# houzhijian/CONE

Measured on AMD Instinct MI355X. Metric: windows/sec + queries/sec, Ego4D-NLQ win_len=90 d=256 top-k=20, higher is better.
Workload: dtype f32

## Files before the change

cone_amd/csrc/ffn.hip:

```cpp
#include <mutex>

#include "tail_f32_common.h"

namespace cone {

constexpr int FFN_STAGE = 2 * 16 * 256;
constexpr int FFN_NST = 4;

template <bool PROJ, bool QKV, int NW, bool PRE = false>
__global__ __launch_bounds__(64 * NW, NW / 4) void ffn_fused_kernel(FfnArgs p) {
    static_assert(!PRE || (PROJ && !QKV), "the pre-norm form is the layer tail");
    constexpr int FFN_ROWS = 16 * NW, FFN_NPIECE = 32 / NW, NT = 64 * NW, HW = NW / 2;
    extern __shared__ __attribute__((aligned(16))) float smem[];
    float* b1s = smem + FFN_NST * FFN_STAGE;
    TF_LAUNCH_ROWS(M, p, 0)
    const int n_tiles = (M + FFN_ROWS - 1) / FFN_ROWS;
    if (n_tiles == 0) return;
    const int G_ = (int)gridDim.x;
    const int full_items = ((n_tiles - 1) / G_) * G_;
    const int rem_rows = M - full_items * FFN_ROWS;
    const int rem_half = (rem_rows + 63) >> 6;
    const bool half_mode = NW == 8 && rem_half <= G_ && 2 * ((rem_rows + FFN_ROWS - 1) / FFN_ROWS) <= G_;
    const int n_items = full_items + (half_mode ? rem_half : (rem_rows + FFN_ROWS - 1) / FFN_ROWS);
    if ((int)blockIdx.x >= n_items) return;
    const int tid = threadIdx.x, lane = tid & 63;
    const int wave = __builtin_amdgcn_readfirstlane(tid >> 6);
    auto wave_row0 = [&](int it) -> int {
        if (it < full_items || !half_mode) return it * FFN_ROWS + wave * 16;
        return wave < 4 ? full_items * FFN_ROWS + (it - full_items) * 64 + wave * 16 : M;
    };
    const int li = lane & 15, lg = lane >> 4;
    const int ff = p.ff, nc = ff >> 4;
    constexpr int NP = PROJ ? 8 : 0;
    const int NQ = QKV ? p.n_qkv >> 5 : 0;
    const int G = NP + nc + NQ;

    float* prm = b1s + ff;
    for (int i = tid; i < (ff >> 2); i += NT)
        reinterpret_cast<f32x4*>(b1s)[i] = reinterpret_cast<const f32x4*>(p.b1)[i];
    if (tid < 64) {
        reinterpret_cast<f32x4*>(prm)[tid] = reinterpret_cast<const f32x4*>(p.b2)[tid];
        reinterpret_cast<f32x4*>(prm + 256)[tid] = reinterpret_cast<const f32x4*>(p.ln_g)[tid];
        reinterpret_cast<f32x4*>(prm + 512)[tid] = reinterpret_cast<const f32x4*>(p.ln_b)[tid];
        if (PROJ) {
            reinterpret_cast<f32x4*>(prm + 768)[tid] = reinterpret_cast<const f32x4*>(p.bo)[tid];
            reinterpret_cast<f32x4*>(prm + 1024)[tid] = reinterpret_cast<const f32x4*>(p.pg)[tid];
            reinterpret_cast<f32x4*>(prm + 1280)[tid] = reinterpret_cast<const f32x4*>(p.pb)[tid];
        }
    }
    float* qbs = prm + 1536;
    if (QKV)
        for (int i = tid; i < (p.n_qkv >> 2); i += NT)
            reinterpret_cast<f32x4*>(qbs)[i] = reinterpret_cast<const f32x4*>(p.qb)[i];

    const int drow = lane >> 2;
    const int dch = (lane & 3) ^ tf_swz16(drow);
    const bool w2side = wave >= HW;
    const float* fbase = w2side ? p.W2 : p.W1;
    const int foff = w2side ? (16 * FFN_NPIECE * (wave - HW) + drow) * ff + 4 * dch
                            : drow * 256 + 16 * FFN_NPIECE * wave + 4 * dch;
    const int fpiece = w2side ? 16 * ff : 16;
    const int fchunk = w2side ? 16 : 16 * 256;
    const int poff = PROJ ? (16 * (wave / HW) + drow) * 256 + 16 * FFN_NPIECE * (wave % HW) + 4 * dch : 0;
    int sb = 0;
    auto stream_piece = [&](int g, int i) {
        float* dstp = smem + ((sb + g) % FFN_NST) * FFN_STAGE + (wave * FFN_NPIECE + i) * 256;
        const int gg = g < G ? g : g - G;
        const bool qk = QKV && gg >= NP + nc;
        const bool pj = (PROJ && gg < NP) || qk;
        const char* ub = reinterpret_cast<const char*>(
            qk ? p.Wq + ((size_t)(gg - NP - nc) * (32 * 256) + 16 * i)
               : (pj ? p.Wo + ((size_t)gg * (32 * 256) + 16 * i) : fbase + ((size_t)(gg - NP) * fchunk + (size_t)i * fpiece)));
        const unsigned vo = (unsigned)((pj ? poff : foff) * 4);
        asm volatile("" : "+s"(ub));
        TF_GLDS16(ub + vo, dstp);
    };

    const int rd = li * 16 + ((lg ^ tf_swz16(li)) << 2);
#define FFN_RD(stg, off) (*reinterpret_cast<const f32x4*>((stg) + (off) + rd))
#define FFN_STAGE_OF(g) (smem + ((sb + (g)) % FFN_NST) * FFN_STAGE)
#define FFN_SB() __builtin_amdgcn_sched_barrier(0)
#define FFN_STREAM(g, u) { if (FFN_NPIECE == 8) stream_piece(g, u); else if ((u) & 1) stream_piece(g, (u) >> 1); }
#define FFN_END_CHUNK()                                                           \
    {                                                                             \
        FFN_SB();                                                                 \
        asm volatile("s_waitcnt vmcnt(%0)" ::"n"(FFN_NPIECE) : "memory");         \
        __builtin_amdgcn_s_barrier();                                             \
        FFN_SB();                                                                 \
    }
#define FFN_MFMA(acc, a, b) { acc = __builtin_amdgcn_mfma_f32_16x16x4f32(a, b, acc, 0, 0, 0); FFN_SB(); }
#define FFN_MM_A(acc, w0, w1, B, q)                                                   \
    {                                                                                 \
        _Pragma("unroll") for (int r = 0; r < 4; ++r) FFN_MFMA(acc[r], w0[r], B[q][r])         \
        _Pragma("unroll") for (int r = 0; r < 4; ++r) FFN_MFMA(acc[r], w1[r], B[(q) + 1][r])   \
    }
#define FFN_MM_Y(w0, w1, hh, t)                                                       \
    {                                                                                 \
        _Pragma("unroll") for (int r = 0; r < 4; ++r) {                               \
            FFN_MFMA(y[t], w0[r], hh[r])                                              \
            FFN_MFMA(y[(t) + 1], w1[r], hh[r])                                        \
        }                                                                             \
    }
#define FFN_MM_AY(acc, w0, w1, B, q, v0, v1, hh, t)                                   \
    {                                                                                 \
        _Pragma("unroll") for (int r = 0; r < 4; ++r) {                               \
            FFN_MFMA(acc[r], w0[r], B[q][r])                                          \
            FFN_MFMA(y[(t) + (r & 1)], ((r & 1) ? v1 : v0)[r >> 1], hh[r >> 1])       \
        }                                                                             \
        _Pragma("unroll") for (int r = 0; r < 4; ++r) {                               \
            FFN_MFMA(acc[r], w1[r], B[(q) + 1][r])                                    \
            FFN_MFMA(y[(t) + (r & 1)], ((r & 1) ? v1 : v0)[2 + (r >> 1)], hh[2 + (r >> 1)]) \
        }                                                                             \
    }

#define FFN_CHUNK32(gi, B)                                                                                                 \
    const float* st = FFN_STAGE_OF(gi);                                                                                    \
    f32x4 ha[2], hb[2];                                                                                                    \
    ha[0] = f32x4{0.f, 0.f, 0.f, 0.f}; hb[0] = ha[0];                                                                      \
    ha[1] = ha[0]; hb[1] = ha[0];                                                                                          \
    wa = FFN_RD(st, 0); wb = FFN_RD(st, 256); va = FFN_RD(st, 4096); vb = FFN_RD(st, 4096 + 256);                          \
    _Pragma("unroll") for (int u = 0; u < 8; ++u) {                                                                        \
        FFN_SB();                                                                                                          \
        asm volatile("" : "+v"(wa), "+v"(wb), "+v"(va), "+v"(vb));                                                         \
        FFN_SB();                                                                                                          \
        if (u < 7) {                                                                                                       \
            na = FFN_RD(st, (2 * u + 2) * 256); nb = FFN_RD(st, (2 * u + 3) * 256);                                        \
            nva = FFN_RD(st, 4096 + (2 * u + 2) * 256); nvb = FFN_RD(st, 4096 + (2 * u + 3) * 256);                        \
        }                                                                                                                  \
        FFN_SB();                                                                                                          \
        _Pragma("unroll") for (int r = 0; r < 4; ++r) {                                                                    \
            FFN_MFMA(ha[r & 1], wa[r], B[2 * u][r])                                                                        \
            FFN_MFMA(hb[r & 1], va[r], B[2 * u][r])                                                                        \
        }                                                                                                                  \
        _Pragma("unroll") for (int r = 0; r < 4; ++r) {                                                                    \
            FFN_MFMA(ha[r & 1], wb[r], B[2 * u + 1][r])                                                                    \
            FFN_MFMA(hb[r & 1], vb[r], B[2 * u + 1][r])                                                                    \
        }                                                                                                                  \
        FFN_STREAM((gi) + 2, u)                                     \
        if (u < 7) { wa = na; wb = nb; va = nva; vb = nvb; }                                                               \
    }

#pragma unroll
    for (int i = 0; i < FFN_NPIECE; ++i) stream_piece(0, i);
#pragma unroll
    for (int i = 0; i < FFN_NPIECE; ++i) stream_piece(1 < G ? 1 : 0, i);

    f32x4 wa, wb, na, nb;
    f32x4 va, vb, nva, nvb;

    f32x4 xr[16];
    f32x4 ar[PROJ ? 16 : 1];
    auto load_tile = [&](int tile) {
        const int row = wave_row0(tile) + li;
        const size_t ld_row = TF_LD_ROW(row, M);
        if (PROJ) {
            const float* ap = p.A + ld_row * p.lda + 4 * lg;
#pragma unroll
            for (int q = 0; q < 16; ++q) ar[q] = *reinterpret_cast<const f32x4*>(ap + 16 * q);
        } else {
            const float* xp = p.X + ld_row * p.ldx + 4 * lg;
#pragma unroll
            for (int q = 0; q < 16; ++q) xr[q] = *reinterpret_cast<const f32x4*>(xp + 16 * q);
        }
    };
    auto load_res = [&](int tile) {
        const int row = wave_row0(tile) + li;
        const size_t ld_row = TF_LD_ROW(row, M);
        TF_RES_ROW(rp, p, ld_row, 4 * lg)
#pragma unroll
        for (int q = 0; q < 16; ++q) xr[q] = *reinterpret_cast<const f32x4*>(rp + 16 * q);
    };
    load_tile(blockIdx.x);
    bool first = true;
    for (int tile = blockIdx.x; tile < n_items; tile += gridDim.x) {
    const int my_row0 = wave_row0(tile);
    const int my_row = my_row0 + li;
    const bool act = my_row0 < M;
    if (first) {
        asm volatile("s_waitcnt vmcnt(%0)" ::"n"(FFN_NPIECE) : "memory");
        __syncthreads();
        first = false;
    }
    if (!act) {
        for (int g = 0; g < G; ++g) {
#pragma unroll
            for (int i = 0; i < FFN_NPIECE; ++i) stream_piece(g + 2, i);
            FFN_END_CHUNK()
        }
        break;
    }

    f32x4 y[16];
    if (PROJ) {
        load_res(tile);
#pragma unroll
        for (int g = 0; g < NP; ++g) {
            FFN_CHUNK32(g, ar)
            xr[2 * g] += ha[0] + ha[1];
            xr[2 * g + 1] += hb[0] + hb[1];
            FFN_END_CHUNK()
        }
        FFN_SB();
#pragma unroll
        for (int t = 0; t < 16; ++t) xr[t] += *reinterpret_cast<const f32x4*>(prm + 768 + 16 * t + 4 * lg);
        if (PRE) {
#pragma unroll
            for (int t = 0; t < 16; ++t) y[t] = xr[t] + *reinterpret_cast<const f32x4*>(prm + 16 * t + 4 * lg);
        }
        float rstd;
        tf_layernorm_regs(xr, rstd);
        TF_LN_APPLY(xr, rstd, prm + 1024, prm + 1280)
        FFN_SB();
    }

    if (!PRE) {
#pragma unroll
        for (int t = 0; t < 16; ++t) y[t] = f32x4{0.f, 0.f, 0.f, 0.f};
    }
    f32x4 h, hp[4];
    {
        const float* st = FFN_STAGE_OF(NP);
#pragma unroll
        for (int r = 0; r < 4; ++r) hp[r] = f32x4{0.f, 0.f, 0.f, 0.f};
        wa = FFN_RD(st, 0); wb = FFN_RD(st, 256);
#pragma unroll
        for (int u = 0; u < 8; ++u) {
            FFN_SB();
            asm volatile("" : "+v"(wa), "+v"(wb));
            FFN_SB();
            if (u < 7) { na = FFN_RD(st, (2 * u + 2) * 256); nb = FFN_RD(st, (2 * u + 3) * 256); }
            else { va = FFN_RD(st, 4096); vb = FFN_RD(st, 4096 + 256); }
            FFN_SB();
            FFN_MM_A(hp, wa, wb, xr, 2 * u)
            FFN_STREAM(NP + 2, u)
            if (u < 7) { wa = na; wb = nb; }
        }
        FFN_SB();
        h = (hp[0] + hp[1]) + (hp[2] + hp[3]) + *reinterpret_cast<const f32x4*>(b1s + 4 * lg);
#pragma unroll
        for (int r = 0; r < 4; ++r) h[r] = fmaxf(h[r], 0.f);
        FFN_END_CHUNK()
    }
    for (int i = 1; i < nc; ++i) {
        const float* s1 = FFN_STAGE_OF(NP + i);
        const float* s2 = FFN_STAGE_OF(NP + i - 1);
#pragma unroll
        for (int r = 0; r < 4; ++r) hp[r] = f32x4{0.f, 0.f, 0.f, 0.f};
        wa = FFN_RD(s1, 0); wb = FFN_RD(s1, 256);
#pragma unroll
        for (int u = 0; u < 8; ++u) {
            FFN_SB();
            if (u == 0) {
                asm volatile("" : "+v"(va), "+v"(vb));
                FFN_SB();
                nva = FFN_RD(s2, 4096 + 2 * 256); nvb = FFN_RD(s2, 4096 + 3 * 256);
                FFN_SB();
                FFN_MM_Y(va, vb, h, 0)
                FFN_SB();
                asm volatile("" : "+v"(wa), "+v"(wb));
                FFN_SB();
                na = FFN_RD(s1, 2 * 256); nb = FFN_RD(s1, 3 * 256);
                FFN_SB();
                FFN_MM_A(hp, wa, wb, xr, 0)
            } else {
                asm volatile("" : "+v"(wa), "+v"(wb), "+v"(va), "+v"(vb));
                FFN_SB();
                if (u < 7) {
                    na = FFN_RD(s1, (2 * u + 2) * 256); nb = FFN_RD(s1, (2 * u + 3) * 256);
                    nva = FFN_RD(s2, 4096 + (2 * u + 2) * 256); nvb = FFN_RD(s2, 4096 + (2 * u + 3) * 256);
                } else {
                    nva = FFN_RD(s1, 4096); nvb = FFN_RD(s1, 4096 + 256);
                }
                FFN_SB();
                FFN_MM_AY(hp, wa, wb, xr, 2 * u, va, vb, h, 2 * u)
            }
            FFN_STREAM(NP + i + 2, u)
            if (u < 7) { wa = na; wb = nb; }
            va = nva; vb = nvb;
        }
        FFN_SB();
        h = (hp[0] + hp[1]) + (hp[2] + hp[3]) + *reinterpret_cast<const f32x4*>(b1s + 16 * i + 4 * lg);
#pragma unroll
        for (int r = 0; r < 4; ++r) h[r] = fmaxf(h[r], 0.f);
        FFN_END_CHUNK()
    }
    {
        const float* st = FFN_STAGE_OF(NP + nc - 1);
#pragma unroll
        for (int u = 0; u < 8; ++u) {
            FFN_SB();
            asm volatile("" : "+v"(va), "+v"(vb));
            FFN_SB();
            if (u < 7) { nva = FFN_RD(st, 4096 + (2 * u + 2) * 256); nvb = FFN_RD(st, 4096 + (2 * u + 3) * 256); }
            FFN_SB();
            FFN_MM_Y(va, vb, h, 2 * u)
            if (u < 7) { va = nva; vb = nvb; }
        }
    }
    FFN_SB();
    if (!PRE) {
#pragma unroll
        for (int t = 0; t < 16; ++t) y[t] = y[t] + *reinterpret_cast<const f32x4*>(prm + 16 * t + 4 * lg) + xr[t];
    }
    FFN_SB();
    load_tile(tile + (int)gridDim.x < n_items ? tile + (int)gridDim.x : tile);
    FFN_SB();
    if (PRE && my_row < M) {
        float* op = p.OUT + (size_t)my_row * p.ldo + 4 * lg;
#pragma unroll
        for (int t = 0; t < 16; ++t) *reinterpret_cast<f32x4*>(op + 16 * t) = y[t];
    }
    float rstd;
    if (!PRE || p.OUT2) tf_layernorm_regs(y, rstd);
    if (PRE) {
        if (p.OUT2 && my_row < M) {
            float* op = p.OUT2 + (size_t)my_row * p.ldo2 + 4 * lg;
            TF_LN_STORE(op, y, rstd, prm + 256, prm + 512, true, false)
        }
    } else if (my_row < M) {
        float* op = p.OUT + (size_t)my_row * p.ldo + 4 * lg;
        TF_LN_STORE(op, y, rstd, prm + 256, prm + 512, true, QKV)
    } else if (QKV) {
#pragma unroll
        for (int t = 0; t < 16; ++t) y[t] = f32x4{0.f, 0.f, 0.f, 0.f};
    }
    if (QKV) {
        float* qrow = p.QKV + (size_t)my_row * p.ldq + 4 * lg;
        for (int g = 0; g < NQ; ++g) {
            FFN_CHUNK32(NP + nc + g, y)
            FFN_SB();
            if (my_row < M) {
                *reinterpret_cast<f32x4*>(qrow + 32 * g) = (ha[0] + ha[1]) + *reinterpret_cast<const f32x4*>(qbs + 32 * g + 4 * lg);
                *reinterpret_cast<f32x4*>(qrow + 32 * g + 16) = (hb[0] + hb[1]) + *reinterpret_cast<const f32x4*>(qbs + 32 * g + 16 + 4 * lg);
            }
            FFN_END_CHUNK()
        }
    }
    sb = (sb + G) % FFN_NST;
    }
    asm volatile("s_waitcnt vmcnt(0)" ::: "memory");
}

#undef FFN_CHUNK32
#undef FFN_MM_A
#undef FFN_MM_Y
#undef FFN_MM_AY
#undef FFN_MFMA
#undef FFN_END_CHUNK
#undef FFN_SB
#undef FFN_STREAM
#undef FFN_STAGE_OF
#undef FFN_RD

bool ffn_fused_supported(int ff) { return ff >= 32 && ff % 16 == 0 && ff <= 4096; }

bool ffn_fused_qkv_fits(int ff, int n_qkv) {
    return ffn_fused_supported(ff) && n_qkv >= 32 && n_qkv % 32 == 0 &&
           (size_t)(FFN_NST * FFN_STAGE + ff + 6 * 256 + n_qkv) * sizeof(float) <= 160 * 1024;
}

static int ffn_cu_count(int* n_cu) {
    static DeviceOnce once;
    CONE_CHECK_HIP(device_once(once, [] { return hipSuccess; }, n_cu));
    return 0;
}

template <bool PROJ, bool QKV, int NW, bool PRE = false>
static int launch_ffn_nw(const TailF32Args& a, int n_cu, hipStream_t s) {
    const size_t lds = (size_t)(FFN_NST * FFN_STAGE + a.ff + 6 * 256 + (QKV ? a.n_qkv : 0)) * sizeof(float);
    CONE_REQUIRE(lds <= 160 * 1024, "fused layer tail: %zu bytes of LDS (ff %d, q|k|v %d) exceed 160 KiB", lds, a.ff, a.n_qkv);
    static DeviceOnce once;
    int dev_cu = 0;
    CONE_CHECK_HIP(device_once(once, [] {
        return hipFuncSetAttribute((const void*)ffn_fused_kernel<PROJ, QKV, NW, PRE>, hipFuncAttributeMaxDynamicSharedMemorySize,
                                   160 * 1024);
    }, &dev_cu));
    if (!n_cu) n_cu = dev_cu;
    const int tiles = (a.M + 16 * NW - 1) / (16 * NW);
    const int grid = tiles < n_cu ? tiles : n_cu;
    ProfScope ps(NW == 8 ? (PROJ ? PK_FFN_PROJ : PK_FFN_FUSED) : (PROJ ? PK_FFN_PROJ_NW4 : PK_FFN_FUSED_NW4), a.M,
                 a.ff + (QKV ? a.n_qkv / 2 : 0), 256, a.M_dev, s);
    FfnArgs k;
    static_cast<TailF32Args&>(k) = a;
    hipLaunchKernelGGL((ffn_fused_kernel<PROJ, QKV, NW, PRE>), dim3((unsigned)grid), dim3(64 * NW), lds, s, k);
    CONE_LAUNCH_CHECK();
    return 0;
}

static int launch_ffn_rows(const TailF32Args& a, bool proj, bool pre, int nw, int n_cu, hipStream_t s) {
    if (pre) return launch_ffn_nw<true, false, 8, true>(a, n_cu, s);
    if (a.Wq) return launch_ffn_nw<true, true, 8>(a, n_cu, s);
    if (nw == 4) return proj ? launch_ffn_nw<true, false, 4>(a, n_cu, s) : launch_ffn_nw<false, false, 4>(a, n_cu, s);
    return proj ? launch_ffn_nw<true, false, 8>(a, n_cu, s) : launch_ffn_nw<false, false, 8>(a, n_cu, s);
}

#ifndef CONE_FFN_SPLIT_GROUPS
#define CONE_FFN_SPLIT_GROUPS 512
#endif
static int ffn_full_round_rows(int M, int n_cu, int ff) {
    const int tiles = (M + 127) / 128;
    if (tiles <= n_cu || !ffn_wide_supported(ff)) return M;
    const int64_t full = (int64_t)(tiles / n_cu) * n_cu * 128;
    const int64_t rem = M - full;
    return rem > 0 && (rem + 15) / 16 <= CONE_FFN_SPLIT_GROUPS ? (int)full : M;
}

static int launch_ffn_ladder(TailF32Args a, bool proj, int n_cu, int wide_groups, hipStream_t s) {
    const int M = a.M;
    const bool ride = a.Wq != nullptr;
    if (!ride && (M + 15) / 16 <= wide_groups && ffn_wide_supported(a.ff)) return launch_tail_f32_wide(a, proj, false, s);
    if (!n_cu)
        if (int rc = ffn_cu_count(&n_cu)) return rc;
    const int m1 = ride ? M : ffn_full_round_rows(M, n_cu, a.ff);
    a.M = m1;
    if (int rc = launch_ffn_rows(a, proj, false, !ride && 2 * ((m1 + 127) / 128) <= n_cu ? 4 : 8, n_cu, s)) return rc;
    if (m1 == M) return 0;
    a.M = M - m1; a.m_off = m1; a.OUT += (size_t)m1 * a.ldo;
    if (!proj) a.X += (size_t)m1 * a.ldx;
    else {
        a.A += (size_t)m1 * a.lda;
        if (a.r_idx) a.r_idx += m1; else a.R += (size_t)m1 * a.ldr;
    }
    return launch_tail_f32_wide(a, proj, false, s);
}

int launch_ffn_fused(const float* X, int ldx, const float* W1, const float* b1, const float* W2, const float* b2,
                     const float* ln_g, const float* ln_b, float* OUT, int ldo, int M, const int* M_dev, int ff,
                     hipStream_t s) {
    CONE_REQUIRE(ffn_fused_supported(ff), "fused FFN: dim_feedforward=%d unsupported", ff);
    CONE_REQUIRE(X && W1 && b1 && W2 && b2 && ln_g && ln_b && OUT, "fused FFN: null argument");
    CONE_REQUIRE(ldx % 4 == 0 && ldo % 4 == 0, "fused FFN: row strides must be multiples of 4");
    if (M <= 0) return 0;
    TailF32Args a{};
    a.X = X; a.ldx = ldx; a.W1 = W1; a.b1 = b1; a.W2 = W2; a.b2 = b2; a.ln_g = ln_g; a.ln_b = ln_b;
    a.OUT = OUT; a.ldo = ldo; a.M = M; a.M_dev = M_dev; a.ff = ff;
    return launch_ffn_ladder(a, false, 0, FFN_WIDE_GROUPS, s);
}

int launch_proj_ffn_fused(const TailArgs& t, hipStream_t s) {
    if (int rc = tail_f32_check(t, TF_FORM_ROWS, "fused layer tail")) return rc;
    if (t.M <= 0) return 0;
    return launch_ffn_ladder(tail_f32_args(t), true, 0, FFN_WIDE_GROUPS, s);
}

int launch_proj_ffn_prenorm(const TailArgs& t, hipStream_t s) {
    if (int rc = tail_f32_check(t, TF_FORM_ROWS, "pre-norm layer tail")) return rc;
    if (t.M <= 0) return 0;
    return launch_ffn_rows(tail_f32_args(t), true, true, 8, 0, s);
}

int launch_tail_f32_form(const TailArgs& t, int form, int n_cu, hipStream_t s) {
    if (form == CONE_TAIL_FORM_SPREAD) return launch_proj_ffn_spread(t, s);
    CONE_REQUIRE(form >= CONE_TAIL_FORM_ROWS128 && form <= CONE_TAIL_FORM_LADDER, "tail form hook: unknown form %d", form);
    CONE_REQUIRE(!t.pre || (form != CONE_TAIL_FORM_ROWS64 && form != CONE_TAIL_FORM_LADDER), "tail form hook: no such pre-norm form");
    CONE_REQUIRE(form != CONE_TAIL_FORM_LADDER || n_cu > 0, "tail form hook: the ladder needs a CU count");
    if (int rc = tail_f32_check(t, form == CONE_TAIL_FORM_WIDE ? TF_FORM_WIDE : TF_FORM_ROWS, "tail form hook")) return rc;
    if (t.M <= 0) return 0;
    const TailF32Args a = tail_f32_args(t);
    if (form == CONE_TAIL_FORM_WIDE) return launch_tail_f32_wide(a, true, t.pre, s);
    if (form == CONE_TAIL_FORM_LADDER) return launch_ffn_ladder(a, true, n_cu, 0, s);
    return launch_ffn_rows(a, true, t.pre, form == CONE_TAIL_FORM_ROWS64 ? 4 : 8, 0, s);
}
}
```

cone_amd/csrc/tail_f32_common.h:

```cpp
#pragma once

#include "common.h"

namespace cone {

#define TF_GLDS16(src, dst) \
    __builtin_amdgcn_global_load_lds((const __attribute__((address_space(1))) void*)(src), \
                                     (__attribute__((address_space(3))) void*)(dst), 16, 0, 0)

__device__ __forceinline__ int tf_swz16(int row) { return (0x1230 >> (((row >> 2) & 3) * 4)) & 3; }

__device__ __forceinline__ void tf_layernorm_regs(f32x4 (&v)[16], float& rstd) {
    float s1 = 0.f;
#pragma unroll
    for (int t = 0; t < 16; ++t) s1 += (v[t][0] + v[t][1]) + (v[t][2] + v[t][3]);
    s1 += __shfl_xor(s1, 16, 64);
    s1 += __shfl_xor(s1, 32, 64);
    const float mean = s1 * (1.0f / 256.0f);
    float s2 = 0.f;
#pragma unroll
    for (int t = 0; t < 16; ++t) {
#pragma unroll
        for (int r = 0; r < 4; ++r) { v[t][r] -= mean; s2 = fmaf(v[t][r], v[t][r], s2); }
    }
    s2 += __shfl_xor(s2, 16, 64);
    s2 += __shfl_xor(s2, 32, 64);
    rstd = 1.0f / sqrtf(s2 * (1.0f / 256.0f) + 1e-5f);
}
#define TF_LN_TILE(o, v, rstd, gp, bp, t)                                                       \
    {                                                                                           \
        const f32x4 g_ = *reinterpret_cast<const f32x4*>((gp) + 16 * (t) + 4 * lg);             \
        const f32x4 b_ = *reinterpret_cast<const f32x4*>((bp) + 16 * (t) + 4 * lg);             \
        _Pragma("unroll") for (int r = 0; r < 4; ++r) o[r] = v[t][r] * rstd * g_[r] + b_[r];    \
    }
#define TF_LN_APPLY(v, rstd, gp, bp) \
    _Pragma("unroll") for (int t = 0; t < 16; ++t) TF_LN_TILE(v[t], v, rstd, gp, bp, t)
#define TF_LN_STORE(op, v, rstd, gp, bp, WHEN, KEEP)             \
    _Pragma("unroll") for (int t = 0; t < 16; ++t) {             \
        if (WHEN) {                                              \
            f32x4 o_;                                            \
            TF_LN_TILE(o_, v, rstd, gp, bp, t)                   \
            *reinterpret_cast<f32x4*>((op) + 16 * t) = o_;       \
            if (KEEP) v[t] = o_;                                 \
        }                                                        \
    }

#define TF_LAUNCH_ROWS(M, p, m_off) \
    int M = (p).M;                  \
    if ((p).M_dev) { const int md_ = *(p).M_dev - (m_off); M = md_ < M ? md_ : M; }
#define TF_LD_ROW(row, M) ((size_t)((row) < (M) ? (row) : (M) - 1))
#define TF_RES_ROW(rp, p, ld_row, off)                                                                               \
    const float* rp = (p).R + (ld_row) * (p).ldr + (off);                                                            \
    if ((p).r_idx) {                                                                                                 \
        const int ix_ = (p).r_idx[ld_row];                                                                           \
        rp = (ix_ >= 0 ? (p).R + (size_t)ix_ * (p).ldr : (p).R2 + (size_t)(~ix_) * (p).ldr) + (off);                 \
    }

struct TailF32Args {
    const float* X; int ldx;
    const float* W1; const float* b1;
    const float* W2; const float* b2;
    const float* ln_g; const float* ln_b;
    float* OUT; int ldo;
    int M; const int* M_dev;
    int ff;
    const float* A; int lda; const float* R; int ldr;
    const float* Wo; const float* bo; const float* pg; const float* pb;
    const int* r_idx; const float* R2;
    const float* Wq; const float* qb; float* QKV; int ldq; int n_qkv;
    float* OUT2; int ldo2;
    int m_off;
};
struct FfnArgs : TailF32Args {};
struct FfnWideArgs : TailF32Args {};

enum { TF_FORM_ROWS = 0, TF_FORM_WIDE = 1, TF_FORM_SPREAD = 2 };

bool ffn_fused_supported(int ff);
bool ffn_wide_supported(int ff);
bool ffn_spread_supported(int M, int ff);

static inline bool tail_f32_rides(const TailArgs& t) { return !t.pre && t.next && t.next->Wq; }

static inline TailF32Args tail_f32_args(const TailArgs& t) {
    const TailWeights& w = *t.w;
    TailF32Args a{};
    a.A = t.A; a.lda = t.lda; a.Wo = w.Wo; a.bo = w.bo; a.R = t.R; a.ldr = t.ldr; a.pg = w.in_g; a.pb = w.in_b;
    a.r_idx = t.r_idx; a.R2 = t.R2;
    a.W1 = w.W1; a.b1 = w.b1; a.W2 = w.W2; a.b2 = w.b2;
    a.ln_g = t.pre && !w.out_g ? w.in_g : w.out_g; a.ln_b = t.pre && !w.out_b ? w.in_b : w.out_b;
    a.OUT = t.OUT; a.ldo = t.ldo; a.M = t.M; a.M_dev = t.M_dev; a.ff = t.ff; a.m_off = t.m_off;
    if (t.pre) { a.OUT2 = t.OUT2; a.ldo2 = t.ldo2; }
    if (tail_f32_rides(t)) { a.Wq = t.next->Wq; a.qb = t.next->qb; a.QKV = t.QKV; a.ldq = t.ldq; a.n_qkv = t.n_qkv; }
    return a;
}

static inline int tail_f32_check(const TailArgs& t, int form, const char* what) {
    const TailWeights& w = *t.w;
    CONE_REQUIRE(form != TF_FORM_SPREAD || (ffn_spread_supported(t.M, t.ff) && t.scratch), "%s: unsupported size M=%d ff=%d", what,
                 t.M, t.ff);
    CONE_REQUIRE(!t.r_idx || t.R2, "%s: a gathered residual needs both source matrices", what);
    CONE_REQUIRE(form == TF_FORM_SPREAD || (form == TF_FORM_WIDE ? ffn_wide_supported(t.ff) : ffn_fused_supported(t.ff)),
                 "%s: dim_feedforward=%d unsupported", what, t.ff);
    CONE_REQUIRE(t.A && w.Wo && w.bo && t.R && w.in_g && w.in_b && w.W1 && w.b1 && w.W2 && w.b2 && t.OUT &&
                     (t.pre ? !t.OUT2 || (w.out_g && w.out_b) : w.out_g && w.out_b), "%s: null argument", what);
    CONE_REQUIRE(t.lda % 4 == 0 && t.ldr % 4 == 0 && t.ldo % 4 == 0 && (!t.pre || !t.OUT2 || t.ldo2 % 4 == 0),
                 "%s: row strides must be multiples of 4", what);
    CONE_REQUIRE(form != TF_FORM_ROWS || !tail_f32_rides(t) ||
                     (t.next->qb && t.QKV && t.n_qkv >= 32 && t.n_qkv % 32 == 0 && t.ldq % 4 == 0), "%s: bad q|k|v arguments", what);
    return 0;
}

int launch_tail_f32_wide(const TailF32Args& a, bool proj, bool pre, hipStream_t s);
int launch_tail_f32_spread(const TailF32Args& a, bool pre, float* scratch, hipStream_t s);

}
```

Measured before the change: 375,000.

## Prefetch activation and residual rows with counted vmcnt waits in fused FFN

Row loads for the attention output, residual and input now go through inline global_load asm, and the kernel waits on them with explicit vmcnt counts that leave younger stores and weight streams in flight. The residual gather index is fetched together with the attention rows, and the next tile's attention load is issued earlier for the non-QKV projection path. The intent is to overlap these row loads with the MFMA chunks instead of stalling on full waits. The q|k|v ride path drops to a single accumulator pair. Compile-time ablation macros that disable output stores are added but default off. The hand-counted vmcnt values are fragile: a miscount could read data before it lands.

```diff
diff --git a/cone_amd/csrc/ffn.hip b/cone_amd/csrc/ffn.hip
--- a/cone_amd/csrc/ffn.hip
+++ b/cone_amd/csrc/ffn.hip
@@ -3,6 +3,20 @@
 #include "tail_f32_common.h"
 
 namespace cone {
+
+#ifndef CONE_FFN_ABL_NO_OUT_STORES
+#define CONE_FFN_ABL_NO_OUT_STORES 0
+#endif
+#ifndef CONE_FFN_ABL_NO_RIDE_STORES
+#define CONE_FFN_ABL_NO_RIDE_STORES 0
+#endif
+#ifndef CONE_FFN_STRICT_WAIT
+#define CONE_FFN_STRICT_WAIT 0
+#endif
+constexpr bool FFN_ABL_NO_OUT_STORES = CONE_FFN_ABL_NO_OUT_STORES, FFN_ABL_NO_RIDE_STORES = CONE_FFN_ABL_NO_RIDE_STORES,
+               FFN_STRICT_WAIT = CONE_FFN_STRICT_WAIT;
+#define FFN_OUT_ST(p) (!FFN_ABL_NO_OUT_STORES || (p).ldo < 0)
+#define FFN_RIDE_ST(p) (!FFN_ABL_NO_RIDE_STORES || (p).ldq < 0)
 
 constexpr int FFN_STAGE = 2 * 16 * 256;
 constexpr int FFN_NST = 4;
@@ -81,12 +95,13 @@
 #define FFN_STAGE_OF(g) (smem + ((sb + (g)) % FFN_NST) * FFN_STAGE)
 #define FFN_SB() __builtin_amdgcn_sched_barrier(0)
 #define FFN_STREAM(g, u) { if (FFN_NPIECE == 8) stream_piece(g, u); else if ((u) & 1) stream_piece(g, (u) >> 1); }
-#define FFN_END_CHUNK()                                                           \
-    {                                                                             \
-        FFN_SB();                                                                 \
-        asm volatile("s_waitcnt vmcnt(%0)" ::"n"(FFN_NPIECE) : "memory");         \
-        __builtin_amdgcn_s_barrier();                                             \
-        FFN_SB();                                                                 \
+#define FFN_END_CHUNK(younger)                                                              \
+    {                                                                                       \
+        static_assert(FFN_NPIECE + (younger) <= 63, "vmcnt is a 6-bit field");              \
+        FFN_SB();                                                                           \
+        asm volatile("s_waitcnt vmcnt(%0)" ::"n"(FFN_NPIECE + (younger)) : "memory");       \
+        __builtin_amdgcn_s_barrier();                                                       \
+        FFN_SB();                                                                           \
     }
 #define FFN_MFMA(acc, a, b) { acc = __builtin_amdgcn_mfma_f32_16x16x4f32(a, b, acc, 0, 0, 0); FFN_SB(); }
 #define FFN_MM_A(acc, w0, w1, B, q)                                                   \
@@ -113,11 +128,10 @@
         }                                                                             \
     }
 
-#define FFN_CHUNK32(gi, B)                                                                                                 \
+#define FFN_CHUNK32(gi, B, NCH)                                                                                            \
     const float* st = FFN_STAGE_OF(gi);                                                                                    \
-    f32x4 ha[2], hb[2];                                                                                                    \
-    ha[0] = f32x4{0.f, 0.f, 0.f, 0.f}; hb[0] = ha[0];                                                                      \
-    ha[1] = ha[0]; hb[1] = ha[0];                                                                                          \
+    f32x4 ha[NCH], hb[NCH];                                                                                                \
+    _Pragma("unroll") for (int c_ = 0; c_ < (NCH); ++c_) { ha[c_] = f32x4{0.f, 0.f, 0.f, 0.f}; hb[c_] = ha[c_]; }          \
     wa = FFN_RD(st, 0); wb = FFN_RD(st, 256); va = FFN_RD(st, 4096); vb = FFN_RD(st, 4096 + 256);                          \
     _Pragma("unroll") for (int u = 0; u < 8; ++u) {                                                                        \
         FFN_SB();                                                                                                          \
@@ -129,12 +143,12 @@
         }                                                                                                                  \
         FFN_SB();                                                                                                          \
         _Pragma("unroll") for (int r = 0; r < 4; ++r) {                                                                    \
-            FFN_MFMA(ha[r & 1], wa[r], B[2 * u][r])                                                                        \
-            FFN_MFMA(hb[r & 1], va[r], B[2 * u][r])                                                                        \
+            FFN_MFMA(ha[r & ((NCH) - 1)], wa[r], B[2 * u][r])                                                              \
+            FFN_MFMA(hb[r & ((NCH) - 1)], va[r], B[2 * u][r])                                                              \
         }                                                                                                                  \
         _Pragma("unroll") for (int r = 0; r < 4; ++r) {                                                                    \
-            FFN_MFMA(ha[r & 1], wb[r], B[2 * u + 1][r])                                                                    \
-            FFN_MFMA(hb[r & 1], vb[r], B[2 * u + 1][r])                                                                    \
+            FFN_MFMA(ha[r & ((NCH) - 1)], wb[r], B[2 * u + 1][r])                                                          \
+            FFN_MFMA(hb[r & ((NCH) - 1)], vb[r], B[2 * u + 1][r])                                                          \
         }                                                                                                                  \
         FFN_STREAM((gi) + 2, u)                                     \
         if (u < 7) { wa = na; wb = nb; va = nva; vb = nvb; }                                                               \
@@ -148,36 +162,55 @@
     f32x4 wa, wb, na, nb;
     f32x4 va, vb, nva, nvb;
 
+    constexpr int ROWS = 16, OUT_ST = FFN_ABL_NO_OUT_STORES ? 0 : 16, RIDE_ST = FFN_ABL_NO_RIDE_STORES ? 0 : 2;
+    constexpr int AR_WAIT = FFN_STRICT_WAIT ? 0 : OUT_ST + (QKV ? FFN_NPIECE + RIDE_ST : 0);
+    constexpr int XR_WAIT = FFN_STRICT_WAIT ? 0 : PROJ ? FFN_NPIECE : OUT_ST;
+    constexpr int END0_YOUNGER = FFN_STRICT_WAIT || PROJ ? 0 : OUT_ST;
+    constexpr int RIDE_YOUNGER = FFN_STRICT_WAIT ? 0 : 2 * RIDE_ST, RIDE0_YOUNGER = FFN_STRICT_WAIT ? 0 : ROWS + OUT_ST + RIDE_ST;
     f32x4 xr[16];
     f32x4 ar[PROJ ? 16 : 1];
-    auto load_tile = [&](int tile) {
-        const int row = wave_row0(tile) + li;
-        const size_t ld_row = TF_LD_ROW(row, M);
-        if (PROJ) {
-            const float* ap = p.A + ld_row * p.lda + 4 * lg;
-#pragma unroll
-            for (int q = 0; q < 16; ++q) ar[q] = *reinterpret_cast<const f32x4*>(ap + 16 * q);
-        } else {
-            const float* xp = p.X + ld_row * p.ldx + 4 * lg;
-#pragma unroll
-            for (int q = 0; q < 16; ++q) xr[q] = *reinterpret_cast<const f32x4*>(xp + 16 * q);
-        }
+    int gix = 0;
+#define FFN_LD1(v, ptr, q) asm volatile("global_load_dwordx4 %0, %1, off offset:" #q "*64 ; rows " #v : "=v"(v[q]) : "v"(ptr) : "memory");
+#define FFN_LDROWS(v, ptr)                                                                                                 \
+    {                                                                                                                      \
+        FFN_SB();                                                                                                          \
+        FFN_LD1(v, ptr, 0) FFN_LD1(v, ptr, 1) FFN_LD1(v, ptr, 2) FFN_LD1(v, ptr, 3) FFN_LD1(v, ptr, 4) FFN_LD1(v, ptr, 5)  \
+        FFN_LD1(v, ptr, 6) FFN_LD1(v, ptr, 7) FFN_LD1(v, ptr, 8) FFN_LD1(v, ptr, 9) FFN_LD1(v, ptr, 10) FFN_LD1(v, ptr, 11) \
+        FFN_LD1(v, ptr, 12) FFN_LD1(v, ptr, 13) FFN_LD1(v, ptr, 14) FFN_LD1(v, ptr, 15)                                    \
+        FFN_SB();                                                                                                          \
+    }
+#define FFN_WAIT_ROWS(v, n)                                                                                                \
+    {                                                                                                                      \
+        static_assert((n) <= 63, "vmcnt is a 6-bit field");                                                                \
+        FFN_SB();                                                                                                          \
+        asm volatile("s_waitcnt vmcnt(%8) ; landed " #v : "+v"(v[0]), "+v"(v[1]), "+v"(v[2]), "+v"(v[3]), "+v"(v[4]), "+v"(v[5]),       \
+                     "+v"(v[6]), "+v"(v[7]) : "n"(n) : "memory");                                                          \
+        asm volatile("" : "+v"(v[8]), "+v"(v[9]), "+v"(v[10]), "+v"(v[11]), "+v"(v[12]), "+v"(v[13]), "+v"(v[14]),         \
+                     "+v"(v[15]) :: "memory");                                                                             \
+        FFN_SB();                                                                                                          \
+    }
+    auto ld_row_of = [&](int it) -> size_t { return TF_LD_ROW(wave_row0(it) + li, M); };
+    auto load_attn = [&](int it) {
+        const size_t ld_row = ld_row_of(it);
+        const int* ip = p.r_idx ? p.r_idx + ld_row : reinterpret_cast<const int*>(p.A);
+        const float* ap = p.A + ld_row * p.lda + 4 * lg;
+        FFN_SB();
+        asm volatile("global_load_dword %0, %1, off ; rows ar" : "=v"(gix) : "v"(ip) : "memory");
+        FFN_LDROWS(ar, ap)
     };
-    auto load_res = [&](int tile) {
-        const int row = wave_row0(tile) + li;
-        const size_t ld_row = TF_LD_ROW(row, M);
-        TF_RES_ROW(rp, p, ld_row, 4 * lg)
-#pragma unroll
-        for (int q = 0; q < 16; ++q) xr[q] = *reinterpret_cast<const f32x4*>(rp + 16 * q);
-    };
-    load_tile(blockIdx.x);
+    if (PROJ) load_attn(blockIdx.x);
+    else {
+        const float* xp = p.X + ld_row_of(blockIdx.x) * p.ldx + 4 * lg;
+        FFN_LDROWS(xr, xp)
+    }
     bool first = true;
     for (int tile = blockIdx.x; tile < n_items; tile += gridDim.x) {
     const int my_row0 = wave_row0(tile);
     const int my_row = my_row0 + li;
     const bool act = my_row0 < M;
+    const int nxt = tile + (int)gridDim.x < n_items ? tile + (int)gridDim.x : tile;
     if (first) {
-        asm volatile("s_waitcnt vmcnt(%0)" ::"n"(FFN_NPIECE) : "memory");
+        asm volatile("s_waitcnt vmcnt(0)" ::: "memory");
         __syncthreads();
         first = false;
     }
@@ -185,20 +218,34 @@
         for (int g = 0; g < G; ++g) {
 #pragma unroll
             for (int i = 0; i < FFN_NPIECE; ++i) stream_piece(g + 2, i);
-            FFN_END_CHUNK()
+            FFN_END_CHUNK(0)
         }
         break;
     }
 
     f32x4 y[16];
     if (PROJ) {
-        load_res(tile);
+        FFN_WAIT_ROWS(ar, AR_WAIT)
+        asm volatile("" : "+v"(gix));
+        FFN_SB();
+        {
+            const size_t ld_row = ld_row_of(tile);
+            TF_RES_ROW_IX(rp, p, ld_row, 4 * lg, gix)
+            FFN_LDROWS(xr, rp)
+        }
 #pragma unroll
         for (int g = 0; g < NP; ++g) {
-            FFN_CHUNK32(g, ar)
+            FFN_CHUNK32(g, ar, 2)
+            if (g == 0) {
+                FFN_WAIT_ROWS(xr, XR_WAIT)
+            }
             xr[2 * g] += ha[0] + ha[1];
             xr[2 * g + 1] += hb[0] + hb[1];
-            FFN_END_CHUNK()
+            if (g == 0) {
+                FFN_END_CHUNK(END0_YOUNGER)
+            } else {
+                FFN_END_CHUNK(0)
+            }
         }
         FFN_SB();
 #pragma unroll
@@ -213,6 +260,9 @@
         FFN_SB();
     }
 
+    if (!PROJ) {
+        FFN_WAIT_ROWS(xr, XR_WAIT)
+    }
     if (!PRE) {
 #pragma unroll
         for (int t = 0; t < 16; ++t) y[t] = f32x4{0.f, 0.f, 0.f, 0.f};
@@ -239,7 +289,11 @@
         h = (hp[0] + hp[1]) + (hp[2] + hp[3]) + *reinterpret_cast<const f32x4*>(b1s + 4 * lg);
 #pragma unroll
         for (int r = 0; r < 4; ++r) h[r] = fmaxf(h[r], 0.f);
-        FFN_END_CHUNK()
+        if (PROJ) {
+            FFN_END_CHUNK(0)
+        } else {
+            FFN_END_CHUNK(END0_YOUNGER)
+        }
     }
     for (int i = 1; i < nc; ++i) {
         const float* s1 = FFN_STAGE_OF(NP + i);
@@ -282,8 +336,9 @@
         h = (hp[0] + hp[1]) + (hp[2] + hp[3]) + *reinterpret_cast<const f32x4*>(b1s + 16 * i + 4 * lg);
 #pragma unroll
         for (int r = 0; r < 4; ++r) h[r] = fmaxf(h[r], 0.f);
-        FFN_END_CHUNK()
-    }
+        FFN_END_CHUNK(0)
+    }
+    if (PROJ && !QKV) load_attn(nxt);
     {
         const float* st = FFN_STAGE_OF(NP + nc - 1);
 #pragma unroll
@@ -303,9 +358,14 @@
         for (int t = 0; t < 16; ++t) y[t] = y[t] + *reinterpret_cast<const f32x4*>(prm + 16 * t + 4 * lg) + xr[t];
     }
     FFN_SB();
-    load_tile(tile + (int)gridDim.x < n_items ? tile + (int)gridDim.x : tile);
+    if (!PROJ) {
+        const float* xp = p.X + ld_row_of(nxt) * p.ldx + 4 * lg;
+        FFN_LDROWS(xr, xp)
+    } else if (QKV) {
+        load_attn(nxt);
+    }
     FFN_SB();
-    if (PRE && my_row < M) {
+    if (PRE && my_row < M && FFN_OUT_ST(p)) {
         float* op = p.OUT + (size_t)my_row * p.ldo + 4 * lg;
 #pragma unroll
         for (int t = 0; t < 16; ++t) *reinterpret_cast<f32x4*>(op + 16 * t) = y[t];
@@ -315,11 +375,11 @@
     if (PRE) {
         if (p.OUT2 && my_row < M) {
             float* op = p.OUT2 + (size_t)my_row * p.ldo2 + 4 * lg;
-            TF_LN_STORE(op, y, rstd, prm + 256, prm + 512, true, false)
+            TF_LN_STORE(op, y, rstd, prm + 256, prm + 512, FFN_OUT_ST(p), false)
         }
     } else if (my_row < M) {
         float* op = p.OUT + (size_t)my_row * p.ldo + 4 * lg;
-        TF_LN_STORE(op, y, rstd, prm + 256, prm + 512, true, QKV)
+        TF_LN_STORE(op, y, rstd, prm + 256, prm + 512, FFN_OUT_ST(p), QKV)
     } else if (QKV) {
 #pragma unroll
         for (int t = 0; t < 16; ++t) y[t] = f32x4{0.f, 0.f, 0.f, 0.f};
@@ -327,13 +387,17 @@
     if (QKV) {
         float* qrow = p.QKV + (size_t)my_row * p.ldq + 4 * lg;
         for (int g = 0; g < NQ; ++g) {
-            FFN_CHUNK32(NP + nc + g, y)
-            FFN_SB();
-            if (my_row < M) {
-                *reinterpret_cast<f32x4*>(qrow + 32 * g) = (ha[0] + ha[1]) + *reinterpret_cast<const f32x4*>(qbs + 32 * g + 4 * lg);
-                *reinterpret_cast<f32x4*>(qrow + 32 * g + 16) = (hb[0] + hb[1]) + *reinterpret_cast<const f32x4*>(qbs + 32 * g + 16 + 4 * lg);
+            FFN_CHUNK32(NP + nc + g, y, 1)
+            FFN_SB();
+            if (my_row < M && FFN_RIDE_ST(p)) {
+                *reinterpret_cast<f32x4*>(qrow + 32 * g) = ha[0] + *reinterpret_cast<const f32x4*>(qbs + 32 * g + 4 * lg);
+                *reinterpret_cast<f32x4*>(qrow + 32 * g + 16) = hb[0] + *reinterpret_cast<const f32x4*>(qbs + 32 * g + 16 + 4 * lg);
             }
-            FFN_END_CHUNK()
+            if (g == 0) {
+                FFN_END_CHUNK(RIDE0_YOUNGER)
+            } else {
+                FFN_END_CHUNK(RIDE_YOUNGER)
+            }
         }
     }
     sb = (sb + G) % FFN_NST;
@@ -342,6 +406,9 @@
 }
 
 #undef FFN_CHUNK32
+#undef FFN_LD1
+#undef FFN_LDROWS
+#undef FFN_WAIT_ROWS
 #undef FFN_MM_A
 #undef FFN_MM_Y
 #undef FFN_MM_AY
diff --git a/cone_amd/csrc/tail_f32_common.h b/cone_amd/csrc/tail_f32_common.h
--- a/cone_amd/csrc/tail_f32_common.h
+++ b/cone_amd/csrc/tail_f32_common.h
@@ -49,10 +49,11 @@
     int M = (p).M;                  \
     if ((p).M_dev) { const int md_ = *(p).M_dev - (m_off); M = md_ < M ? md_ : M; }
 #define TF_LD_ROW(row, M) ((size_t)((row) < (M) ? (row) : (M) - 1))
-#define TF_RES_ROW(rp, p, ld_row, off)                                                                               \
+#define TF_RES_ROW(rp, p, ld_row, off) TF_RES_ROW_IX(rp, p, ld_row, off, (p).r_idx[ld_row])
+#define TF_RES_ROW_IX(rp, p, ld_row, off, IX)                                                                        \
     const float* rp = (p).R + (ld_row) * (p).ldr + (off);                                                            \
     if ((p).r_idx) {                                                                                                 \
-        const int ix_ = (p).r_idx[ld_row];                                                                           \
+        const int ix_ = (IX);                                                                                        \
         rp = (ix_ >= 0 ? (p).R + (size_t)ix_ * (p).ldr : (p).R2 + (size_t)(~ix_) * (p).ldr) + (off);                 \
     }
 
```

Result: no change. 377,700, median of 6 (+0.7%).
